# uzh-rpg/dagr

Measured on NVIDIA H100. Metric: Mevents/sec, higher is better.
Workload: dtype f32

## Files before the change

### dagr_b200/csrc/graph.cu

```cuda
#include "common.cuh"

#define SCAN_THREADS 256
#define SCAN_ITEMS 8
#define SCAN_TILE (SCAN_THREADS * SCAN_ITEMS)

extern "C" int64_t dagr_scan_blocks(int64_t n) { return (n + SCAN_TILE - 1) / SCAN_TILE; }

__global__ void __launch_bounds__(SCAN_THREADS) k_scan_reduce(const int *__restrict__ in, int64_t n, int *__restrict__ blocksums)
{
    __shared__ int sm[32];
    __shared__ int tot;
    int64_t base = (int64_t)blockIdx.x * SCAN_TILE + (int64_t)threadIdx.x * SCAN_ITEMS;
    int s = 0;
#pragma unroll
    for (int k = 0; k < SCAN_ITEMS; k++) { int64_t i = base + k; if (i < n) s += in[i]; }
    block_exclusive_scan(s, &tot, sm);
    if (threadIdx.x == 0) blocksums[blockIdx.x] = tot;
}

__global__ void __launch_bounds__(SCAN_THREADS) k_scan_blocksums(int *__restrict__ blocksums, int64_t nb)
{
    __shared__ int sm[32];
    __shared__ int tot;
    int carry = 0;
    for (int64_t c = 0; c < nb; c += SCAN_THREADS) {
        int64_t i = c + threadIdx.x;
        int v = (i < nb) ? blocksums[i] : 0;
        int ex = block_exclusive_scan(v, &tot, sm);
        if (i < nb) blocksums[i] = ex + carry;
        carry += tot;
        __syncthreads();
    }
    if (threadIdx.x == 0) blocksums[nb] = carry;
}

__global__ void __launch_bounds__(SCAN_THREADS) k_scan_apply(const int *__restrict__ in, int *__restrict__ out, int64_t n,
                                                             const int *__restrict__ blocksums, int64_t nb)
{
    __shared__ int sm[32];
    __shared__ int tot;
    int64_t base = (int64_t)blockIdx.x * SCAN_TILE + (int64_t)threadIdx.x * SCAN_ITEMS;
    int v[SCAN_ITEMS];
    int s = 0;
#pragma unroll
    for (int k = 0; k < SCAN_ITEMS; k++) { int64_t i = base + k; v[k] = (i < n) ? in[i] : 0; s += v[k]; }
    int ex = block_exclusive_scan(s, &tot, sm) + blocksums[blockIdx.x];
#pragma unroll
    for (int k = 0; k < SCAN_ITEMS; k++) { int64_t i = base + k; if (i < n) out[i] = ex; ex += v[k]; }
    if (blockIdx.x == 0 && threadIdx.x == 0) out[n] = blocksums[nb];
}

int scan_exclusive(const int *in, int *out, int64_t n, int *blocksums, cudaStream_t st)
{
    int64_t nb = dagr_scan_blocks(n);
    if (nb == 0) nb = 1;
    k_scan_reduce<<<(unsigned)nb, SCAN_THREADS, 0, st>>>(in, n, blocksums);
    k_scan_blocksums<<<1, SCAN_THREADS, 0, st>>>(blocksums, nb);
    k_scan_apply<<<(unsigned)nb, SCAN_THREADS, 0, st>>>(in, out, n, blocksums, nb);
    return 0;
}

__global__ void k_denorm(const float *__restrict__ pos, int64_t n3, float W, float H, float T, int32_t *__restrict__ out)
{
    int64_t i = (int64_t)blockIdx.x * blockDim.x + threadIdx.x;
    if (i >= n3) return;
    int d = (int)(i % 3);
    float s = d == 0 ? W : (d == 1 ? H : T);
    out[i] = (int)__fadd_rn(__fmul_rn(s, pos[i]), 1e-3f);
}

extern "C" int dagr_denormalize_pos(const float *pos, int64_t N, int W, int H, int T, int32_t *pos_i32, void *stream)
{
    if (N <= 0) return DAGR_OK;
    int64_t n3 = 3 * N;
    k_denorm<<<dagr_div_up(n3, 256), 256, 0, (cudaStream_t)stream>>>(pos, n3, (float)W, (float)H, (float)T, pos_i32);
    DAGR_CHECK_LAUNCH();
    return DAGR_OK;
}

__global__ void k_prepare_events(const float *__restrict__ pos, const int64_t *__restrict__ batch64, const float *__restrict__ x, int ldx,
                                 int64_t N, float W, float H, float T, int32_t *__restrict__ pos_i, int32_t *__restrict__ batch_i,
                                 float *__restrict__ feat)
{
    const int64_t i = (int64_t)blockIdx.x * blockDim.x + threadIdx.x;
    if (i >= N) return;
    pos_i[3 * i + 0] = (int)__fadd_rn(__fmul_rn(W, pos[3 * i + 0]), 1e-3f);
    pos_i[3 * i + 1] = (int)__fadd_rn(__fmul_rn(H, pos[3 * i + 1]), 1e-3f);
    pos_i[3 * i + 2] = (int)__fadd_rn(__fmul_rn(T, pos[3 * i + 2]), 1e-3f);
    batch_i[i] = (int32_t)batch64[i];
    feat[i] = x[i * ldx];
}

extern "C" int dagr_prepare_events(const float *pos, const int64_t *batch, const float *x, int ldx, int64_t N, int W, int H, int T,
                                   int32_t *pos_i32, int32_t *batch_i32, float *feat, void *stream)
{
    if (N <= 0) return DAGR_OK;
    DAGR_CHECK_ARG(pos && batch && x && pos_i32 && batch_i32 && feat && ldx >= 1, "bad argument");
    k_prepare_events<<<dagr_div_up(N, 256), 256, 0, (cudaStream_t)stream>>>(pos, batch, x, ldx, N, (float)W, (float)H, (float)T, pos_i32,
                                                                          batch_i32, feat);
    DAGR_CHECK_LAUNCH();
    return DAGR_OK;
}

struct RingAt {
    int64_t slot;
    int i;
};

__device__ __forceinline__ int64_t ring_total(const int32_t *ctl, int S, int64_t N)
{
    if (ctl == nullptr) return N;
    return S == 1 ? (int64_t)ctl[1] : (int64_t)ctl[DAGR_RING_CTL * S];
}

__device__ __forceinline__ RingAt ring_at(const int32_t *ctl, int S, int mask, int c)
{
    if (ctl == nullptr) return RingAt{(int64_t)c, c};
    int s = 0;
    if (S > 1) {
        int lo = 0, hi = S - 1;
        while (lo < hi) {
            const int mid = (lo + hi + 1) >> 1;
            if (__ldg(ctl + DAGR_RING_CTL * mid + 6) <= c) lo = mid; else hi = mid - 1;
        }
        s = lo;
    }
    const int32_t *cs = ctl + DAGR_RING_CTL * s;
    const int i = S > 1 ? c - __ldg(cs + 6) : c;
    return RingAt{(int64_t)s * (mask + 1) + ((__ldg(cs) + i) & mask), i};
}

__global__ void k_keys_hist(dagr_geom_t g, const int32_t *__restrict__ batch, const int32_t *__restrict__ pos, int64_t N,
                            int32_t *__restrict__ key, int32_t *__restrict__ count, int32_t *__restrict__ flags,
                            const int32_t *__restrict__ ctl, int mask, int S)
{
    int64_t i = (int64_t)blockIdx.x * blockDim.x + threadIdx.x;
    if (i >= ring_total(ctl, S, N)) return;
    const RingAt at = ring_at(ctl, S, mask, (int)i);
    const int64_t si = at.slot;
    int x = pos[3 * si], y = pos[3 * si + 1], b = batch[si];
    if (flags != nullptr && at.i > 0) {
        const int64_t sp = ctl != nullptr ? (si & ~(int64_t)mask) | ((si - 1) & mask) : si - 1;
        if (batch[sp] == b && pos[3 * sp + 2] > pos[3 * si + 2]) flags[0] = 1;
    }
    x = min(max(x, 0), g.W - 1); y = min(max(y, 0), g.H - 1); b = min(max(b, 0), g.B - 1);
    int k = b * (g.ny1 * g.nx1 * g.CP) + __ldg(g.ykey + y) + __ldg(g.xkey + x);
    key[i] = k;
    atomicAdd(count + k, 1);
}

__global__ void k_scatter(const int32_t *__restrict__ key, int64_t N, const int32_t *__restrict__ start,
                          int32_t *__restrict__ count, int32_t *__restrict__ tmp, const int32_t *__restrict__ ctl, int S)
{
    int64_t i = (int64_t)blockIdx.x * blockDim.x + threadIdx.x;
    if (i >= ring_total(ctl, S, N)) return;
    int k = key[i];
    int slot = atomicSub(count + k, 1) - 1;
    tmp[start[k] + slot] = (int)i;
}

__global__ void k_rank_emit(dagr_geom_t g, const int32_t *__restrict__ key, const int32_t *__restrict__ tmp, int64_t N,
                            const int32_t *__restrict__ start, const int32_t *__restrict__ batch,
                            const int32_t *__restrict__ pos, const float *__restrict__ feat,
                            int32_t *__restrict__ perm, int2 *__restrict__ ti, uint32_t *__restrict__ xyb,
                            float *__restrict__ feat_s, const int32_t *__restrict__ ctl, int mask, int S)
{
    int64_t j = (int64_t)blockIdx.x * blockDim.x + threadIdx.x;
    if (j >= ring_total(ctl, S, N)) return;
    int i = tmp[j];
    int k = key[i];
    int s = start[k], e = start[k + 1];
    int rank = 0;
    for (int q = s; q < e; q++) rank += (tmp[q] < i);
    int p = s + rank;
    const int64_t si = ring_at(ctl, S, mask, i).slot;
    int x = pos[3 * si], y = pos[3 * si + 1], t = pos[3 * si + 2], b = batch[si];
    x = min(max(x, 0), g.W - 1); y = min(max(y, 0), g.H - 1); b = min(max(b, 0), g.B - 1);
    perm[p] = i;
    ti[p] = make_int2(t, i);
    xyb[p] = (uint32_t)x | ((uint32_t)y << 12) | ((uint32_t)b << 24);
    feat_s[p] = feat[si];
}

static int graph_sort_impl(const dagr_geom_t *g, const int32_t *batch, const int32_t *pos, const float *feat,
                           int64_t N, const int32_t *ctl, int mask, int S, int32_t *key, int32_t *tmp, int32_t *count,
                           int32_t *blocksums, int32_t *start, int32_t *perm, int32_t *ti, uint32_t *xyb, float *feat_s,
                           int32_t *flags, void *stream)
{
    DAGR_CHECK_ARG(g && g->W <= 4096 && g->H <= 4096 && g->B <= 256, "geometry out of range (W,H<=4096, B<=256)");
    DAGR_CHECK_ARG(N >= 0 && N < (1ll << 31), "N out of range");
    cudaStream_t st = (cudaStream_t)stream;
    if (N > 0) {
        k_keys_hist<<<dagr_div_up(N, 256), 256, 0, st>>>(*g, batch, pos, N, key, count, flags, ctl, mask, S);
        DAGR_CHECK_LAUNCH();
    }
    scan_exclusive(count, start, g->NK, blocksums, st);
    DAGR_CHECK_LAUNCH();
    if (N > 0) {
        k_scatter<<<dagr_div_up(N, 256), 256, 0, st>>>(key, N, start, count, tmp, ctl, S);
        k_rank_emit<<<dagr_div_up(N, 256), 256, 0, st>>>(*g, key, tmp, N, start, batch, pos, feat, perm,
                                                         (int2 *)ti, xyb, feat_s, ctl, mask, S);
        DAGR_CHECK_LAUNCH();
    }
    return DAGR_OK;
}

extern "C" int dagr_graph_sort(const dagr_geom_t *g, const int32_t *batch, const int32_t *pos, const float *feat,
                               int64_t N, int32_t *key, int32_t *tmp, int32_t *count, int32_t *blocksums,
                               int32_t *start, int32_t *perm, int32_t *ti, uint32_t *xyb, float *feat_s,
                               int32_t *flags, void *stream)
{
    return graph_sort_impl(g, batch, pos, feat, N, nullptr, 0, 1, key, tmp, count, blocksums, start, perm, ti, xyb, feat_s, flags,
                           stream);
}

#define RING_MAX_STREAMS 128
static int check_rings(const char *who, int64_t capacity, int streams, int max_chunk)
{
    const char *msg = nullptr;
    if (streams < 1 || streams >= RING_MAX_STREAMS) msg = "streams must be in [1, 127]";
    else if (capacity <= 0 || (capacity & (capacity - 1)) != 0) msg = "ring capacity must be a power of two";
    else if ((int64_t)streams * capacity >= (1ll << 24)) msg = "streams * capacity must be < 2^24 (sorted positions are packed in 24 bits)";
    else if (max_chunk <= 0 || max_chunk > capacity) msg = "max_chunk must be in [1, capacity]";
    if (msg == nullptr) return DAGR_OK;
    dagr_set_error("%s: %s", who, msg);
    return DAGR_E_ARG;
}

extern "C" int dagr_graph_sort_ring(const dagr_geom_t *g, const int32_t *batch, const int32_t *pos, const float *feat,
                                    int64_t capacity, const int32_t *ctl, int32_t *key, int32_t *tmp, int32_t *count,
                                    int32_t *blocksums, int32_t *start, int32_t *perm, int32_t *ti, uint32_t *xyb, float *feat_s,
                                    int32_t *flags, void *stream)
{
    DAGR_CHECK_ARG(ctl != nullptr && capacity > 0 && (capacity & (capacity - 1)) == 0, "ring capacity must be a power of two");
    return graph_sort_impl(g, batch, pos, feat, capacity, ctl, (int)(capacity - 1), 1, key, tmp, count, blocksums, start, perm, ti,
                           xyb, feat_s, flags, stream);
}

extern "C" int dagr_graph_sort_rings(const dagr_geom_t *g, const int32_t *batch, const int32_t *pos, const float *feat,
                                     int64_t capacity, int streams, const int32_t *ctl, int32_t *key, int32_t *tmp, int32_t *count,
                                     int32_t *blocksums, int32_t *start, int32_t *perm, int32_t *ti, uint32_t *xyb, float *feat_s,
                                     int32_t *flags, void *stream)
{
    DAGR_CHECK_ARG(g && batch && pos && feat && ctl && key && tmp && count && blocksums && start && perm && ti && xyb && feat_s,
                   "null argument");
    const int rc = check_rings(__func__, capacity, streams, 1);
    if (rc != DAGR_OK) return rc;
    DAGR_CHECK_ARG(streams == g->B, "streams must equal the geometry's batch size B (stream s is sample s)");
    return graph_sort_impl(g, batch, pos, feat, (int64_t)streams * capacity, ctl, (int)(capacity - 1), streams, key, tmp, count,
                           blocksums, start, perm, ti, xyb, feat_s, flags, stream);
}

__global__ void __launch_bounds__(RING_MAX_STREAMS) k_stream_advance(int32_t *__restrict__ ctl, const int32_t *__restrict__ stage,
// ... 196 lines not shown
```

### dagr_b200/csrc/conv_l1.cu

```cuda
#include <string.h>
#include "common.cuh"

#define L1_THREADS 128

struct L1Smem {
    float *tab;
    float *posx;
    float *posy;
    short *sp;
};

__device__ __forceinline__ L1Smem l1_smem_init(const dagr_geom_t &g, const float *__restrict__ tab, unsigned char *raw)
{
    L1Smem s;
    s.tab = (float *)raw;
    s.posx = s.tab + g.ncell * DAGR_TABW;
    s.posy = s.posx + g.W;
    s.sp = (short *)(s.posy + g.H);
    for (int i = threadIdx.x; i < g.ncell * DAGR_TABW; i += blockDim.x) s.tab[i] = tab[i];
    for (int i = threadIdx.x; i < g.W; i += blockDim.x) s.posx[i] = g.posx0[i];
    for (int i = threadIdx.x; i < g.H; i += blockDim.x) s.posy[i] = g.posy0[i];
    for (int i = threadIdx.x; i < g.ncell; i += blockDim.x)
        s.sp[i] = (short)(((int)g.spiral[2 * i] & 0xff) | ((int)g.spiral[2 * i + 1] << 8));
    __syncthreads();
// ... 379 lines not shown
            const float4 wya = *reinterpret_cast<const float4 *>(wyb + yo);
            const float wy4 = *reinterpret_cast<const float *>(wy4b + (yo >> 2));
            CB2_EDGE_FMA();
        }
    } else {
#pragma unroll 1
        for (int q = -1; q < n; q++) {
            int row, dxi, dyi;
            if (q < 0) { row = p; dxi = r; dyi = r; }
            else {
                row = nbr[(int64_t)q * N + p];
                const uint32_t d = s_sp[off[(int64_t)q * N + p]];
                dxi = (int)(d & 31u); dyi = (int)(d >> 5);
            }
            const int sw = XA_SWZ(row);
            const float4 *src = reinterpret_cast<const float4 *>(xa + ((int64_t)half * N + row) * 8);
            const float4 t0 = src[sw], t1 = src[sw ^ 1];
            const float wx = s_wx[grp * 32 + dxi];
            const float4 wya = s_wy[dyi];
            const float wy4 = s_wy4[dyi];
            CB2_EDGE_FMA();
        }
    }
#undef CB2_EDGE_FMA
    if constexpr (TC) {
        const float4 *wf = wfrag + ((size_t)half * CB2_TC_KSTEPS * 32 + (threadIdx.x & 31)) * 2;
        float2 c2[8];
#pragma unroll
        for (int i = 0; i < 8; i++) c2[i] = make_float2(0.f, 0.f);
#pragma unroll
        for (int j = 0; j < CB2_G; j++) {
            const float a[8] = {A[j][0].x, A[j][0].y, A[j][1].x, A[j][1].y, A[j][2].x, A[j][2].y, A[j][3].x, A[j][3].y};
            cb2_tc_kstep(xt, a, wf + (grp + 3 * j) * 64, c2);
        }
#pragma unroll
        for (int i = 0; i < 8; i++) o2[i] = make_float2(__fadd_rn(o2[i].x, c2[i].x), __fadd_rn(o2[i].y, c2[i].y));
        return;
    }
#pragma unroll
    for (int j = 0; j < CB2_G; j++)
#pragma unroll
        for (int k = 0; k < 4; k++)
#pragma unroll
            for (int c4 = 0; c4 < 4; c4++) {
                const float4 wa = *reinterpret_cast<const float4 *>(&P.w[grp + 3 * j][8 * half + 2 * k][4 * c4]);
                const float4 wb = *reinterpret_cast<const float4 *>(&P.w[grp + 3 * j][8 * half + 2 * k + 1][4 * c4]);
                o2[2 * c4] = ffma2(make_float2(A[j][k].x, A[j][k].x), make_float2(wa.x, wa.y), o2[2 * c4]);
                o2[2 * c4 + 1] = ffma2(make_float2(A[j][k].x, A[j][k].x), make_float2(wa.z, wa.w), o2[2 * c4 + 1]);
                o2[2 * c4] = ffma2(make_float2(A[j][k].y, A[j][k].y), make_float2(wb.x, wb.y), o2[2 * c4]);
                o2[2 * c4 + 1] = ffma2(make_float2(A[j][k].y, A[j][k].y), make_float2(wb.z, wb.w), o2[2 * c4 + 1]);
            }
}

__device__ __forceinline__ float cb2_div_floor(float a, float b)
{
    const float mod = fmodf(a, b);
    float div = __fdiv_rn(__fsub_rn(a, mod), b);
    if ((mod != 0.f) && ((b < 0.f) != (mod < 0.f))) div -= 1.f;
    float fl;
    if (div != 0.f) { fl = floorf(div); if (div - fl > 0.5f) fl += 1.f; }
    else fl = copysignf(0.f, __fdiv_rn(a, b));
    return fl;
}
__device__ __forceinline__ int cb2_round_to_pixel(float mean, int size)
{
    const float inv = __frcp_rn((float)size);
    const int k = (int)cb2_div_floor(__fadd_rn(mean, 1e-5f), inv);
    return min(max(k, 0), size - 1);
}

template <int THREADS>
struct CB2Shared {
    CB2Tile T;
    uint64_t bar;
    float red[THREADS / 32][16];
    long long sum[THREADS / 32][3];
    int tm[THREADS / 32];
    __align__(16) float xt[THREADS / 32][64];
};

template <class PT, int NCH, bool MODE_A, int CAP, int THREADS, bool POOL_MEAN, bool PLAIN, bool TC>
__device__ __forceinline__ void cb2_voxel(const dagr_geom_t &g, int64_t N, const int32_t *__restrict__ start, const uint32_t *__restrict__ xyb,
             const int2 *__restrict__ ti, const float *__restrict__ feat_s, const float *__restrict__ xa,
             const int32_t *__restrict__ nbr, const uint16_t *__restrict__ off,
             const PT &P, const float4 *__restrict__ wfrag, const float *__restrict__ skip_pre_in, const int min_idx_in,
             float *__restrict__ persist_in, float *__restrict__ x1_in, int32_t *__restrict__ cnt, int32_t *__restrict__ pxy,
             float *__restrict__ tmean, float *__restrict__ tmax, float *__restrict__ xg, int ldx,
             float *__restrict__ xa_out, float *__restrict__ skip_out,
             const int cell, unsigned char *smem_raw, CB2Shared<THREADS> &S, uint32_t &parity,
             int32_t *__restrict__ wl_hdr, int32_t *__restrict__ wl_ids, const int defer)
{
    const int min_idx = PLAIN ? 0 : min_idx_in;
    float *const persist = PLAIN ? nullptr : persist_in;
    float *const x1 = PLAIN ? nullptr : x1_in;
    const float *const skip_pre = PLAIN ? nullptr : skip_pre_in;
    const bool relu = PLAIN ? true : (P.relu != 0);
    CB2Tile &T = S.T;
    uint64_t &s_bar = S.bar;
    auto &s_red = S.red;
    auto &s_sum = S.sum;
    auto &s_tm = S.tm;
    float *const xt = S.xt[threadIdx.x >> 5];
    float *s_rows = (float *)smem_raw;
    float *s_wx = s_rows + (size_t)CAP * 8;
    float4 *s_wy = (float4 *)(s_wx + 128);
    float *s_wy4 = (float *)(s_wy + 32);
    uint32_t *s_ell = (uint32_t *)(s_wy + 64);
    uint16_t *s_sp = (uint16_t *)(s_ell + DAGR_ELL * THREADS);
    const int per = g.ny1 * g.nx1;
    const int b = cell / per, rem = cell % per, cy = rem / g.nx1, cx = rem % g.nx1;
    const int p0 = start[(int64_t)cell * g.CP], p1 = start[(int64_t)(cell + 1) * g.CP];
    const int nown = p1 - p0;
    if (nown == 0) {
        if (MODE_A) return;
        if (threadIdx.x == 0) { cnt[cell] = 0; pxy[2 * cell] = 0; pxy[2 * cell + 1] = 0; tmean[cell] = 0.f; tmax[cell] = 0.f; }
        if (threadIdx.x < 16) xg[(int64_t)cell * ldx + threadIdx.x] = 0.f;
        return;
    }
    if (threadIdx.x < 32) {
        const int clo = max(cx - 1, 0), chi = min(cx + 1, g.nx1 - 1);
        const int lane = threadIdx.x, rr = lane >> 1, ry = cy - 1 + rr;
        int v = 0;
        if (lane < 6 && ry >= 0 && ry < g.ny1)
            v = start[((int64_t)b * per + ry * g.nx1 + ((lane & 1) ? chi + 1 : clo)) * g.CP];
        int o = 0;
#pragma unroll
        for (int k = 0; k < 3; k++) {
            const int s0 = __shfl_sync(0xffffffffu, v, 2 * k), e0 = __shfl_sync(0xffffffffu, v, 2 * k + 1);
            const bool ok = (cy - 1 + k >= 0) && (cy - 1 + k < g.ny1);
            if (lane == 0) { T.run_start[k] = ok ? s0 : 0; T.run_len[k] = ok ? e0 - s0 : 0; T.run_off[k] = o; }
            o += ok ? e0 - s0 : 0;
        }
    }
    for (int i = threadIdx.x; i < 2 * g.r + 1; i += blockDim.x) {
        const float4 tx = __ldg(reinterpret_cast<const float4 *>(g.tabx) + i);
        s_wx[i] = tx.x; s_wx[32 + i] = tx.y; s_wx[64 + i] = tx.z;
        s_wy[i] = __ldg(reinterpret_cast<const float4 *>(g.taby) + 2 * i);
        s_wy4[i] = __ldg(g.taby + 8 * i + 4);
    }
    for (int i = threadIdx.x; i < g.ncell; i += blockDim.x)
        s_sp[i] = (uint16_t)(((int)g.spiral[2 * i] + g.r) | (((int)g.spiral[2 * i + 1] + g.r) << 5));
    __syncthreads();
    const int total = T.run_off[2] + T.run_len[2];
    const bool staged = total <= CAP;
    if (!staged && wl_hdr != nullptr) {
        int slot = 0;
        if (threadIdx.x == 0) slot = atomicAdd(&wl_hdr[0], 1);
        if (defer) { if (threadIdx.x == 0) wl_ids[slot] = cell; return; }
    }
    const int s1 = T.run_start[1];
    const int s2 = T.run_len[2] > 0 ? T.run_start[2] : 0x7fffffff;
    const int d0 = T.run_off[0] - T.run_start[0], d1 = T.run_off[1] - T.run_start[1], d2 = T.run_off[2] - T.run_start[2];

    constexpr bool pool_mean = POOL_MEAN && !MODE_A;
    float m[16];
#pragma unroll
    for (int c = 0; c < 16; c++) m[c] = pool_mean ? 0.f : -INFINITY;
    long long sx = 0, sy = 0, st = 0;
    int tm = -2147483647;
    const bool sparse = MODE_A && staged && nown <= 32;
    const int lane_ = threadIdx.x & 31, wid_ = threadIdx.x >> 5;
    for (int pb0 = p0; pb0 < p1; pb0 += blockDim.x) {
        const int p = sparse ? p0 + lane_ : pb0 + threadIdx.x;
        const bool inrange = sparse ? (p < p1 && wid_ < 3) : (p < p1);
        const int tix = sparse ? lane_ : (int)threadIdx.x;
        const bool active = inrange && (min_idx <= 0 || ti[p].y >= min_idx);
        if (min_idx > 0 && !__syncthreads_or(active)) {
            if (inrange) { const uint32_t w0 = xyb[p]; const int t0 = ti[p].x; sx += w0 & 0xfff; sy += (w0 >> 12) & 0xfff; st += t0; tm = max(tm, t0); }
            continue;
        }
        const int n = active ? nbr[(int64_t)(DAGR_ELL - 1) * N + p] : 0;
        if (staged && active && (!sparse || wid_ == 0)) {
            int jj[DAGR_ELL - 1]; int cc[DAGR_ELL - 1];
#pragma unroll
            for (int q = 0; q < DAGR_ELL - 1; q++) {
                jj[q] = (q < n) ? nbr[(int64_t)q * N + p] : 0;
                cc[q] = (q < n) ? (int)off[(int64_t)q * N + p] : 0;
            }
#pragma unroll
            for (int q = 0; q < DAGR_ELL - 1; q++) {
                const int j = jj[q];
                const int row = j + (j >= s2 ? d2 : (j >= s1 ? d1 : d0));
                s_ell[(q + 1) * THREADS + tix] = ((uint32_t)(2 * row + XA_SWZ(j)) << 4) | ((uint32_t)s_sp[cc[q]] << 18);
            }
            s_ell[tix] = ((uint32_t)(2 * (p + d1) + XA_SWZ(p)) << 4) | ((uint32_t)(g.r | (g.r << 5)) << 18);
        }
        float2 o2[8], sk2[MODE_A ? 8 : 1];
#pragma unroll
        for (int k = 0; k < 8; k++) o2[k] = make_float2(0.f, 0.f);
#pragma unroll
        for (int k = 0; k < (MODE_A ? 8 : 1); k++) sk2[k] = make_float2(0.f, 0.f);
#pragma unroll 1
        for (int half = 0; half < NCH; half++) {
            if (staged) {
                __syncthreads();
                if (threadIdx.x == 0) {
                    mbar_expect_tx(&s_bar, (uint32_t)total * 32u);
                    for (int rr = 0; rr < 3; rr++)
                        if (T.run_len[rr] > 0)
                            tma_bulk_g2s(s_rows + (size_t)T.run_off[rr] * 8, xa + ((size_t)half * N + T.run_start[rr]) * 8,
                                         (uint32_t)T.run_len[rr] * 32u, &s_bar);
                }
                mbar_wait(&s_bar, parity);
                parity ^= 1;
            }
            if (TC ? __any_sync(0xffffffffu, active) : active) {
                const int nn = active ? n : -1;
#define CB2_ROOT(H)                                                                                                  \
    do {                                                                                                            \
        const float4 *src = staged ? reinterpret_cast<const float4 *>(s_rows + (int64_t)(p + d1) * 8)               \
                                   : reinterpret_cast<const float4 *>(xa + ((int64_t)(H) * N + p) * 8);             \
        const float4 z4 = make_float4(0.f, 0.f, 0.f, 0.f);                                                         \
        const float4 t0 = active ? src[XA_SWZ(p)] : z4, t1 = active ? src[XA_SWZ(p) ^ 1] : z4;                      \
        const float v[8] = {t0.x, t0.y, t0.z, t0.w, t1.x, t1.y, t1.z, t1.w};                                        \
        if constexpr (TC) {                                                                                         \
            float2 c2[8];                                                                                           \
            _Pragma("unroll") for (int i = 0; i < 8; i++) c2[i] = make_float2(0.f, 0.f);                            \
            cb2_tc_kstep(xt, v, wfrag + (((H) * CB2_TC_KSTEPS + 15) * 32 + lane_) * 2, c2);                         \
            _Pragma("unroll") for (int i = 0; i < 8; i++)                                                           \
                o2[i] = make_float2(__fadd_rn(o2[i].x, c2[i].x), __fadd_rn(o2[i].y, c2[i].y));                      \
        }                                                                                                           \
        _Pragma("unroll") for (int k = 0; k < 8; k++)                                                               \
            _Pragma("unroll") for (int c4 = 0; c4 < 4; c4++) {                                                      \
                if constexpr (!TC) {                                                                                \
                    const float4 w4 = *reinterpret_cast<const float4 *>(&P.root[8 * (H) + k][4 * c4]);              \
                    o2[2 * c4] = ffma2(make_float2(v[k], v[k]), make_float2(w4.x, w4.y), o2[2 * c4]);               \
                    o2[2 * c4 + 1] = ffma2(make_float2(v[k], v[k]), make_float2(w4.z, w4.w), o2[2 * c4 + 1]);       \
                }                                                                                                   \
                if constexpr (MODE_A) {                     \
                    const float4 k4 = *reinterpret_cast<const float4 *>(&P.skip[8 * (H) + k][4 * c4]);              \
                    sk2[2 * c4] = ffma2(make_float2(v[k], v[k]), make_float2(k4.x, k4.y), sk2[2 * c4]);             \
                    sk2[2 * c4 + 1] = ffma2(make_float2(v[k], v[k]), make_float2(k4.z, k4.w), sk2[2 * c4 + 1]);     \
                }                                                                                                   \
            }                                                                                                       \
    } while (0)
                if (!sparse || wid_ == 0) {
                    if (half == 0)      CB2_ROOT(0);
                    else if (half == 1) CB2_ROOT(1);
                    else if constexpr (NCH > 2) CB2_ROOT(2);
                }
#undef CB2_ROOT
#define CB2_PASS(H, G)                                                                                               \
    do {                                                                                                            \
        if (staged) cb2_pass<true, H, G, THREADS, TC>(N, p, nn, xa, s_rows, s_wx, s_wy, s_wy4, s_ell, s_sp, nbr, off, P, wfrag, xt, p + d1, g.r, tix, o2); \
        else        cb2_pass<false, H, G, THREADS, TC>(N, p, nn, xa, s_rows, s_wx, s_wy, s_wy4, s_ell, s_sp, nbr, off, P, wfrag, xt, 0, g.r, tix, o2);     \
    } while (0)
#define CB2_HALF(H)                                                                                                  \
    do {                                                                                                            \
        if (!sparse) { CB2_PASS(H, 0); CB2_PASS(H, 1); CB2_PASS(H, 2); }                                            \
        else if (wid_ == 0) CB2_PASS(H, 0);                                                                         \
        else if (wid_ == 1) CB2_PASS(H, 1);                                                                         \
        else CB2_PASS(H, 2);                                                                                        \
    } while (0)
                if (half == 0)      CB2_HALF(0);
                else if (half == 1) CB2_HALF(1);
                else if constexpr (NCH > 2) CB2_HALF(2);
#undef CB2_HALF
#undef CB2_PASS
            }
        }
        if constexpr (TC) {
            if (__any_sync(0xffffffffu, active)) cb2_tc_unfrag(xt, o2);
        }
        if (sparse) {
            __syncthreads();
            float *s_part = s_rows;
            if (active && wid_ >= 1) {
                float4 *dst = reinterpret_cast<float4 *>(s_part + ((size_t)(wid_ - 1) * 32 + lane_) * 16);
                dst[0] = make_float4(o2[0].x, o2[0].y, o2[1].x, o2[1].y);
                dst[1] = make_float4(o2[2].x, o2[2].y, o2[3].x, o2[3].y);
                dst[2] = make_float4(o2[4].x, o2[4].y, o2[5].x, o2[5].y);
                dst[3] = make_float4(o2[6].x, o2[6].y, o2[7].x, o2[7].y);
            }
            __syncthreads();
            if (active && wid_ == 0) {
#pragma unroll
                for (int w2 = 0; w2 < 2; w2++) {
                    const float4 *src = reinterpret_cast<const float4 *>(s_part + ((size_t)w2 * 32 + lane_) * 16);
#pragma unroll
                    for (int k = 0; k < 4; k++) {
                        const float4 v = src[k];
                        o2[2 * k].x += v.x; o2[2 * k].y += v.y; o2[2 * k + 1].x += v.z; o2[2 * k + 1].y += v.w;
                    }
                }
            }
        }
        const bool owner = !sparse || wid_ == 0;
        if (!MODE_A && inrange && owner) { const uint32_t w0 = xyb[p]; const int t0 = ti[p].x; sx += w0 & 0xfff; sy += (w0 >> 12) & 0xfff; st += t0; tm = max(tm, t0); }
        if (!active || !owner) continue;
        float o[16];
#pragma unroll
        for (int c = 0; c < 8; c++) { o[2 * c] = o2[c].x; o[2 * c + 1] = o2[c].y; }
        if constexpr (MODE_A) {
            float sk[16];
#pragma unroll
            for (int c = 0; c < 8; c++) { sk[2 * c] = sk2[c].x; sk[2 * c + 1] = sk2[c].y; }
            const int sw = XA_SWZ(p);
            {
                const float4 *pp = reinterpret_cast<const float4 *>(xa_out + (int64_t)p * 8);
                const float4 a0 = pp[sw], a1 = pp[sw ^ 1];
                pp = reinterpret_cast<const float4 *>(xa_out + (N + (int64_t)p) * 8);
                const float4 a2 = pp[sw], a3 = pp[sw ^ 1];
// ... 57 lines not shown
            float4 *dst = reinterpret_cast<float4 *>(x1 + (int64_t)p * 16);
            dst[0] = make_float4(o[0], o[1], o[2], o[3]);
            dst[1] = make_float4(o[4], o[5], o[6], o[7]);
            dst[2] = make_float4(o[8], o[9], o[10], o[11]);
            dst[3] = make_float4(o[12], o[13], o[14], o[15]);
        }
    }
    if (MODE_A) return;
    const int lane = threadIdx.x & 31, wid = threadIdx.x >> 5;
#pragma unroll
    for (int d = 16; d > 0; d >>= 1) {
#pragma unroll
        for (int c = 0; c < 16; c++) {
            const float o2 = __shfl_xor_sync(0xffffffffu, m[c], d);
            m[c] = pool_mean ? m[c] + o2 : fmaxf(m[c], o2);
        }
        sx += __shfl_xor_sync(0xffffffffu, sx, d);
        sy += __shfl_xor_sync(0xffffffffu, sy, d);
        st += __shfl_xor_sync(0xffffffffu, st, d);
        tm = max(tm, __shfl_xor_sync(0xffffffffu, tm, d));
    }
    if (lane == 0) {
#pragma unroll
        for (int c = 0; c < 16; c++) s_red[wid][c] = m[c];
        s_sum[wid][0] = sx; s_sum[wid][1] = sy; s_sum[wid][2] = st; s_tm[wid] = tm;
    }
    __syncthreads();
    const int nw = blockDim.x >> 5;
    if (threadIdx.x < 16) {
        float v = s_red[0][threadIdx.x];
        for (int w2 = 1; w2 < nw; w2++) v = pool_mean ? v + s_red[w2][threadIdx.x] : fmaxf(v, s_red[w2][threadIdx.x]);
        if (pool_mean) v = __fdiv_rn(v, (float)nown);
        if (persist != nullptr) {
            if (min_idx > 0) v = fmaxf(v, persist[(int64_t)cell * 16 + threadIdx.x]);
            persist[(int64_t)cell * 16 + threadIdx.x] = v;
        }
        xg[(int64_t)cell * ldx + threadIdx.x] = v;
    }
    if (threadIdx.x == 32) {
        long long ax = 0, ay = 0, at = 0; int tmx = -2147483647;
        for (int w2 = 0; w2 < nw; w2++) { ax += s_sum[w2][0]; ay += s_sum[w2][1]; at += s_sum[w2][2]; tmx = max(tmx, s_tm[w2]); }
        const float mx = (float)((double)ax / ((double)nown * (double)g.W));
        const float my = (float)((double)ay / ((double)nown * (double)g.H));
        cnt[cell] = nown;
        pxy[2 * cell] = cb2_round_to_pixel(mx, g.W);
        pxy[2 * cell + 1] = cb2_round_to_pixel(my, g.H);
        tmean[cell] = (float)((double)at / ((double)nown * (double)g.T));
        tmax[cell] = __fdiv_rn((float)tmx, (float)g.T);
    }
}


template <class PT, int NCH, bool MODE_A, bool POOL_MEAN, bool PLAIN, bool TC>
__global__ void __launch_bounds__(CB2_THREADS, MODE_A ? 3 : 4)
k_l1_conv_b2(const dagr_geom_t g, int64_t N, const int32_t *__restrict__ start, const uint32_t *__restrict__ xyb,
             const int2 *__restrict__ ti, const float *__restrict__ feat_s, const float *__restrict__ xa,
             const int32_t *__restrict__ nbr, const uint16_t *__restrict__ off,
             const __grid_constant__ PT P, const float4 *__restrict__ wfrag, const float *__restrict__ skip_pre, const int min_idx,
             float *__restrict__ persist, float *__restrict__ x1, int32_t *__restrict__ cnt, int32_t *__restrict__ pxy,
             float *__restrict__ tmean, float *__restrict__ tmax, float *__restrict__ xg, int ldx,
             float *__restrict__ xa_out, float *__restrict__ skip_out, int32_t *__restrict__ wl_hdr, int32_t *__restrict__ wl_ids,
             const int defer)
{
    extern __shared__ __align__(128) unsigned char smem_raw[];
    __shared__ __align__(16) CB2Shared<CB2_THREADS> S;
    if (threadIdx.x == 0) mbar_init(&S.bar, 1);
    uint32_t parity = 0;
    cb2_voxel<PT, NCH, MODE_A, CB2_CAP, CB2_THREADS, POOL_MEAN, PLAIN, TC>(g, N, start, xyb, ti, feat_s, xa, nbr, off, P, wfrag, skip_pre, min_idx,
                                                      persist, x1, cnt, pxy, tmean, tmax, xg, ldx, xa_out, skip_out, (int)blockIdx.x,
                                                      smem_raw, S, parity, wl_hdr, wl_ids, defer);
}

template <class PT, int NCH, bool MODE_A, bool POOL_MEAN, bool PLAIN, bool TC>
__global__ void __launch_bounds__(CB2_THREADS_BIG, 1)
k_l1_conv_b2_dense(const dagr_geom_t g, int64_t N, const int32_t *__restrict__ start, const uint32_t *__restrict__ xyb,
                   const int2 *__restrict__ ti, const float *__restrict__ feat_s, const float *__restrict__ xa,
                   const int32_t *__restrict__ nbr, const uint16_t *__restrict__ off,
                   const __grid_constant__ PT P, const float4 *__restrict__ wfrag, const float *__restrict__ skip_pre, const int min_idx,
                   float *__restrict__ persist, float *__restrict__ x1, int32_t *__restrict__ cnt, int32_t *__restrict__ pxy,
                   float *__restrict__ tmean, float *__restrict__ tmax, float *__restrict__ xg, int ldx,
                   float *__restrict__ xa_out, float *__restrict__ skip_out, int32_t *__restrict__ wl_hdr, const int32_t *__restrict__ wl_ids)
{
    extern __shared__ __align__(128) unsigned char smem_raw[];
    __shared__ __align__(16) CB2Shared<CB2_THREADS_BIG> S;
    __shared__ int s_next;
    if (threadIdx.x == 0) mbar_init(&S.bar, 1);
    uint32_t parity = 0;
    const int count = wl_hdr[0];
    for (;;) {
        __syncthreads();
        if (threadIdx.x == 0) s_next = atomicAdd(&wl_hdr[1], 1);
        __syncthreads();
        const int i = s_next;
        if (i >= count) break;
        cb2_voxel<PT, NCH, MODE_A, CB2_CAP_BIG, CB2_THREADS_BIG, POOL_MEAN, PLAIN, TC>(g, N, start, xyb, ti, feat_s, xa, nbr, off, P, wfrag, skip_pre,
                                                                  min_idx, persist, x1, cnt, pxy, tmean, tmax, xg, ldx, xa_out, skip_out,
                                                                  wl_ids[i], smem_raw, S, parity, nullptr, nullptr, 0);
    }
}

static size_t cb2_smem_bytes(const dagr_geom_t *g, int cap, int threads)
{
    return (size_t)cap * 32 + 96 * 16 + (size_t)DAGR_ELL * threads * 4 + (size_t)g->ncell * 2 + 32;
}

template <class PT, int NCH, bool MODE_A, bool TC, bool POOL_MEAN = false, bool PLAIN = false>
static int cb2_launch(const dagr_geom_t *g, int64_t N, const int32_t *start, const uint32_t *xyb, const int2 *ti, const float *feat_s,
// ... 164 lines not shown
```

Before: 576.2.

## Vectorize scan I/O and fold bucket cursors into scan output

Scan kernels now load and store each thread's eight items as two int4 accesses when aligned and in bounds. The scan apply step also writes per-bucket end cursors back into the count array, so scatter needs one atomicSub and no lookup of start. The rank/emit kernel resets count to zero per bucket, which may let later calls skip a separate memset, and derives the batch index from the key instead of reading it. The cost is more coupling between kernels: count now carries state from one stage to the next, and in-place aliasing drops the __restrict__ qualifiers.

```diff
diff --git a/dagr_b200/csrc/graph.cu b/dagr_b200/csrc/graph.cu
--- a/dagr_b200/csrc/graph.cu
+++ b/dagr_b200/csrc/graph.cu
@@ -6,14 +6,44 @@
 
 extern "C" int64_t dagr_scan_blocks(int64_t n) { return (n + SCAN_TILE - 1) / SCAN_TILE; }
 
-__global__ void __launch_bounds__(SCAN_THREADS) k_scan_reduce(const int *__restrict__ in, int64_t n, int *__restrict__ blocksums)
+static_assert(SCAN_ITEMS == 8, "a thread's items are two int4");
+
+__device__ __forceinline__ bool scan_vec(const void *p, int64_t base, int64_t n)
+{
+    return base + SCAN_ITEMS <= n && ((uintptr_t)p & 15) == 0;
+}
+__device__ __forceinline__ void scan_load(const int *p, int64_t base, int64_t n, int v[SCAN_ITEMS])
+{
+    if (scan_vec(p, base, n)) {
+        const int4 a = *reinterpret_cast<const int4 *>(p + base), b = *reinterpret_cast<const int4 *>(p + base + 4);
+        v[0] = a.x; v[1] = a.y; v[2] = a.z; v[3] = a.w; v[4] = b.x; v[5] = b.y; v[6] = b.z; v[7] = b.w;
+    } else {
+#pragma unroll
+        for (int k = 0; k < SCAN_ITEMS; k++) v[k] = base + k < n ? p[base + k] : 0;
+    }
+}
+__device__ __forceinline__ void scan_store(int *p, int64_t base, int64_t n, const int v[SCAN_ITEMS])
+{
+    if (scan_vec(p, base, n)) {
+        *reinterpret_cast<int4 *>(p + base) = make_int4(v[0], v[1], v[2], v[3]);
+        *reinterpret_cast<int4 *>(p + base + 4) = make_int4(v[4], v[5], v[6], v[7]);
+    } else {
+#pragma unroll
+        for (int k = 0; k < SCAN_ITEMS; k++)
+            if (base + k < n) p[base + k] = v[k];
+    }
+}
+
+__global__ void __launch_bounds__(SCAN_THREADS) k_scan_reduce(const int *in, int64_t n, int *__restrict__ blocksums)
 {
     __shared__ int sm[32];
     __shared__ int tot;
     int64_t base = (int64_t)blockIdx.x * SCAN_TILE + (int64_t)threadIdx.x * SCAN_ITEMS;
+    int v[SCAN_ITEMS];
+    scan_load(in, base, n, v);
     int s = 0;
 #pragma unroll
-    for (int k = 0; k < SCAN_ITEMS; k++) { int64_t i = base + k; if (i < n) s += in[i]; }
+    for (int k = 0; k < SCAN_ITEMS; k++) s += v[k];
     block_exclusive_scan(s, &tot, sm);
     if (threadIdx.x == 0) blocksums[blockIdx.x] = tot;
 }
@@ -34,29 +64,41 @@
     if (threadIdx.x == 0) blocksums[nb] = carry;
 }
 
-__global__ void __launch_bounds__(SCAN_THREADS) k_scan_apply(const int *__restrict__ in, int *__restrict__ out, int64_t n,
-                                                             const int *__restrict__ blocksums, int64_t nb)
+__global__ void __launch_bounds__(SCAN_THREADS) k_scan_apply(const int *in, int *out, int64_t n, const int *__restrict__ blocksums,
+                                                             int64_t nb, int *cursor)
 {
     __shared__ int sm[32];
     __shared__ int tot;
     int64_t base = (int64_t)blockIdx.x * SCAN_TILE + (int64_t)threadIdx.x * SCAN_ITEMS;
-    int v[SCAN_ITEMS];
+    int v[SCAN_ITEMS], o[SCAN_ITEMS];
+    scan_load(in, base, n, v);
     int s = 0;
 #pragma unroll
-    for (int k = 0; k < SCAN_ITEMS; k++) { int64_t i = base + k; v[k] = (i < n) ? in[i] : 0; s += v[k]; }
+    for (int k = 0; k < SCAN_ITEMS; k++) s += v[k];
     int ex = block_exclusive_scan(s, &tot, sm) + blocksums[blockIdx.x];
 #pragma unroll
-    for (int k = 0; k < SCAN_ITEMS; k++) { int64_t i = base + k; if (i < n) out[i] = ex; ex += v[k]; }
+    for (int k = 0; k < SCAN_ITEMS; k++) { o[k] = ex; ex += v[k]; }
+    scan_store(out, base, n, o);
+    if (cursor != nullptr) {
+#pragma unroll
+        for (int k = 0; k < SCAN_ITEMS; k++) o[k] = v[k] > 0 ? o[k] + v[k] : 0;
+        scan_store(cursor, base, n, o);
+    }
     if (blockIdx.x == 0 && threadIdx.x == 0) out[n] = blocksums[nb];
 }
 
-int scan_exclusive(const int *in, int *out, int64_t n, int *blocksums, cudaStream_t st)
+static void scan_launch(const int *in, int *out, int64_t n, int *blocksums, int *cursor, cudaStream_t st)
 {
     int64_t nb = dagr_scan_blocks(n);
     if (nb == 0) nb = 1;
     k_scan_reduce<<<(unsigned)nb, SCAN_THREADS, 0, st>>>(in, n, blocksums);
     k_scan_blocksums<<<1, SCAN_THREADS, 0, st>>>(blocksums, nb);
-    k_scan_apply<<<(unsigned)nb, SCAN_THREADS, 0, st>>>(in, out, n, blocksums, nb);
+    k_scan_apply<<<(unsigned)nb, SCAN_THREADS, 0, st>>>(in, out, n, blocksums, nb, cursor);
+}
+
+int scan_exclusive(const int *in, int *out, int64_t n, int *blocksums, cudaStream_t st)
+{
+    scan_launch(in, out, n, blocksums, nullptr, st);
     return 0;
 }
 
@@ -149,18 +191,16 @@
     atomicAdd(count + k, 1);
 }
 
-__global__ void k_scatter(const int32_t *__restrict__ key, int64_t N, const int32_t *__restrict__ start,
-                          int32_t *__restrict__ count, int32_t *__restrict__ tmp, const int32_t *__restrict__ ctl, int S)
+__global__ void k_scatter(const int32_t *__restrict__ key, int64_t N, int32_t *__restrict__ count, int32_t *__restrict__ tmp,
+                          const int32_t *__restrict__ ctl, int S)
 {
     int64_t i = (int64_t)blockIdx.x * blockDim.x + threadIdx.x;
     if (i >= ring_total(ctl, S, N)) return;
-    int k = key[i];
-    int slot = atomicSub(count + k, 1) - 1;
-    tmp[start[k] + slot] = (int)i;
+    tmp[atomicSub(count + key[i], 1) - 1] = (int)i;
 }
 
 __global__ void k_rank_emit(dagr_geom_t g, const int32_t *__restrict__ key, const int32_t *__restrict__ tmp, int64_t N,
-                            const int32_t *__restrict__ start, const int32_t *__restrict__ batch,
+                            const int32_t *__restrict__ start, int32_t *__restrict__ count,
                             const int32_t *__restrict__ pos, const float *__restrict__ feat,
                             int32_t *__restrict__ perm, int2 *__restrict__ ti, uint32_t *__restrict__ xyb,
                             float *__restrict__ feat_s, const int32_t *__restrict__ ctl, int mask, int S)
@@ -173,9 +213,11 @@
     int rank = 0;
     for (int q = s; q < e; q++) rank += (tmp[q] < i);
     int p = s + rank;
+    if (rank == 0) count[k] = 0;
     const int64_t si = ring_at(ctl, S, mask, i).slot;
-    int x = pos[3 * si], y = pos[3 * si + 1], t = pos[3 * si + 2], b = batch[si];
-    x = min(max(x, 0), g.W - 1); y = min(max(y, 0), g.H - 1); b = min(max(b, 0), g.B - 1);
+    int x = pos[3 * si], y = pos[3 * si + 1], t = pos[3 * si + 2];
+    const int b = k / (g.ny1 * g.nx1 * g.CP);
+    x = min(max(x, 0), g.W - 1); y = min(max(y, 0), g.H - 1);
     perm[p] = i;
     ti[p] = make_int2(t, i);
     xyb[p] = (uint32_t)x | ((uint32_t)y << 12) | ((uint32_t)b << 24);
@@ -194,11 +236,11 @@
         k_keys_hist<<<dagr_div_up(N, 256), 256, 0, st>>>(*g, batch, pos, N, key, count, flags, ctl, mask, S);
         DAGR_CHECK_LAUNCH();
     }
-    scan_exclusive(count, start, g->NK, blocksums, st);
+    scan_launch(count, start, g->NK, blocksums, count, st);
     DAGR_CHECK_LAUNCH();
     if (N > 0) {
-        k_scatter<<<dagr_div_up(N, 256), 256, 0, st>>>(key, N, start, count, tmp, ctl, S);
-        k_rank_emit<<<dagr_div_up(N, 256), 256, 0, st>>>(*g, key, tmp, N, start, batch, pos, feat, perm,
+        k_scatter<<<dagr_div_up(N, 256), 256, 0, st>>>(key, N, count, tmp, ctl, S);
+        k_rank_emit<<<dagr_div_up(N, 256), 256, 0, st>>>(*g, key, tmp, N, start, count, pos, feat, perm,
                                                          (int2 *)ti, xyb, feat_s, ctl, mask, S);
         DAGR_CHECK_LAUNCH();
     }
```

Result: faster. 584.1, median of 6 (+1.4%).

## Split each event's neighbor gather across lane pairs for the tensor-core L1 conv path

Applied to the files above, without the earlier changes.

Adds a paired-lane path for the staged, tensor-core, non-mode-A case. Each event's gathered neighbor rows are split across two lanes that each handle half of the channels. The path runs two 16-row m-tiles per warp, staging accumulators through a larger swizzled per-warp shared buffer and loading them with ldmatrix x4 before the 3xTF32 MMAs. It also lowers the minimum CTAs per SM in launch bounds from 4 to 3 so the larger register and shared-memory footprint fits. The aim is better lane utilisation and fewer shared-memory transposes, at the cost of lower occupancy and more per-lane loop iterations.

```diff
diff --git a/dagr_b200/csrc/conv_l1.cu b/dagr_b200/csrc/conv_l1.cu
--- a/dagr_b200/csrc/conv_l1.cu
+++ b/dagr_b200/csrc/conv_l1.cu
@@ -455,6 +455,120 @@
             }
 }
 
+#ifndef CB2_LANES
+#define CB2_LANES 2
+#endif
+#ifndef CB2_MIN_CTAS
+#define CB2_MIN_CTAS 3
+#endif
+#ifndef CB2_XT_FLOATS
+#define CB2_XT_FLOATS (CB2_MIN_CTAS >= 4 ? 64 : 128)
+#endif
+template <int half, int THREADS>
+__device__ __forceinline__ void cb2_pair_mtile(int n, int col, const float *s_rows, const float4 *s_wx4, const float4 *s_wy,
+                                               const float *s_wy4, const uint32_t *s_ell, const float4 *__restrict__ wfrag, float *xt,
+                                               float2 c[4])
+{
+    const int lane = threadIdx.x & 31, h = lane & 1;
+    float4 A[DAGR_KU];
+#pragma unroll
+    for (int u = 0; u < DAGR_KU; u++) A[u] = make_float4(0.f, 0.f, 0.f, 0.f);
+    const char *rb = reinterpret_cast<const char *>(s_rows), *wxb = reinterpret_cast<const char *>(s_wx4);
+    const char *wyb = reinterpret_cast<const char *>(s_wy), *wy4b = reinterpret_cast<const char *>(s_wy4);
+    const uint32_t hx = 16u * (uint32_t)h;
+#pragma unroll 1
+    for (int q = 0; q <= n; q++) {
+        const uint32_t ell = s_ell[q * THREADS + col];
+        const uint32_t ro = (ell & 0x3fff0u) ^ hx, xo = (ell >> 14) & 0x1f0u, yo = (ell >> 19) & 0x1f0u;
+        const float4 e = *reinterpret_cast<const float4 *>(rb + ro);
+        const float4 wx4 = *reinterpret_cast<const float4 *>(wxb + xo);
+        const float4 wya = *reinterpret_cast<const float4 *>(wyb + yo);
+        const float wy4 = *reinterpret_cast<const float *>(wy4b + (yo >> 2));
+        const float wx[3] = {wx4.x, wx4.y, wx4.z};
+        const float wy[CB2_G] = {wya.x, wya.y, wya.z, wya.w, wy4};
+#pragma unroll
+        for (int k = 0; k < 3; k++)
+#pragma unroll
+            for (int j = 0; j < CB2_G; j++) {
+                const float w = __fmul_rn(wy[j], wx[k]);
+                float4 &a = A[k + 3 * j];
+                a.x = fmaf(w, e.x, a.x); a.y = fmaf(w, e.y, a.y); a.z = fmaf(w, e.z, a.z); a.w = fmaf(w, e.w, a.w);
+            }
+    }
+    const float4 *wf = wfrag + ((size_t)half * CB2_TC_KSTEPS * 32 + lane) * 2;
+#if CB2_XT_FLOATS >= 128
+    const int i_ = lane >> 1, mrow = 8 * ((lane >> 3) & 1) + (lane & 7), mch = lane >> 4;
+    float *row = xt + 8 * i_ + 4 * (h ^ ((i_ >> 2) & 1));
+    const uint32_t ra = smem_u32(xt + 8 * mrow + 4 * (mch ^ ((mrow >> 2) & 1)));
+#else
+    float *row = xt + 4 * (lane >> 1);
+    const uint32_t ra = smem_u32(xt + 4 * (lane & 15));
+#endif
+#pragma unroll
+    for (int grp = 0; grp < 3; grp++) {
+        float2 c2[4];
+#pragma unroll
+        for (int i = 0; i < 4; i++) c2[i] = make_float2(0.f, 0.f);
+#pragma unroll
+        for (int j = 0; j < CB2_G; j++) {
+            const int u = grp + 3 * j;
+            const float4 w0 = __ldg(wf + u * 64), w1 = __ldg(wf + u * 64 + 1);
+            const uint32_t bh[2][2] = {{__float_as_uint(w0.x), __float_as_uint(w0.y)}, {__float_as_uint(w1.x), __float_as_uint(w1.y)}};
+            const uint32_t bl[2][2] = {{__float_as_uint(w0.z), __float_as_uint(w0.w)}, {__float_as_uint(w1.z), __float_as_uint(w1.w)}};
+            uint32_t ah[4], al[4];
+#if CB2_XT_FLOATS >= 128
+            __syncwarp();
+            *reinterpret_cast<float4 *>(row) = A[u];
+            __syncwarp();
+            ldsm_x4(ra, ah);
+#pragma unroll
+            for (int i = 0; i < 4; i++) tf32_split(ah[i], ah[i], al[i]);
+#else
+#pragma unroll
+            for (int hh = 0; hh < 2; hh++) {
+                __syncwarp();
+                if (h == hh) *reinterpret_cast<float4 *>(row) = A[u];
+                __syncwarp();
+                uint32_t r0, r1;
+                ldsm_x2(ra, r0, r1);
+                tf32_split(r0, ah[2 * hh], al[2 * hh]);
+                tf32_split(r1, ah[2 * hh + 1], al[2 * hh + 1]);
+            }
+#endif
+#pragma unroll
+            for (int nt = 0; nt < 2; nt++) {
+                mma_tf32(c2[2 * nt], c2[2 * nt + 1], al, bh[nt][0], bh[nt][1]);
+                mma_tf32(c2[2 * nt], c2[2 * nt + 1], ah, bl[nt][0], bl[nt][1]);
+                mma_tf32(c2[2 * nt], c2[2 * nt + 1], ah, bh[nt][0], bh[nt][1]);
+            }
+        }
+#pragma unroll
+        for (int i = 0; i < 4; i++) c[i] = make_float2(__fadd_rn(c[i].x, c2[i].x), __fadd_rn(c[i].y, c2[i].y));
+    }
+}
+
+template <int half, int THREADS>
+__device__ __forceinline__ void cb2_pair_half(int nn, const float *s_rows, const float4 *s_wx4, const float4 *s_wy, const float *s_wy4,
+                                              const uint32_t *s_ell, const float4 *__restrict__ wfrag, float *xt, float2 o2[8])
+{
+    const int lane = threadIdx.x & 31;
+#pragma unroll 1
+    for (int mt = 0; mt < 2; mt++) {
+        const int src = 16 * mt + (lane >> 1);
+        const int n = __shfl_sync(0xffffffffu, nn, src);
+        if (!__any_sync(0xffffffffu, n >= 0)) continue;
+        float2 c[4];
+#pragma unroll
+        for (int i = 0; i < 4; i++) c[i] = mt ? o2[4 + i] : o2[i];
+        cb2_pair_mtile<half, THREADS>(n, (int)(threadIdx.x & ~31u) + src, s_rows, s_wx4, s_wy, s_wy4, s_ell, wfrag, xt, c);
+#pragma unroll
+        for (int i = 0; i < 4; i++) {
+            if (mt) o2[4 + i] = c[i];
+            else o2[i] = c[i];
+        }
+    }
+}
+
 __device__ __forceinline__ float cb2_div_floor(float a, float b)
 {
     const float mod = fmodf(a, b);
@@ -479,7 +593,7 @@
     float red[THREADS / 32][16];
     long long sum[THREADS / 32][3];
     int tm[THREADS / 32];
-    __align__(16) float xt[THREADS / 32][64];
+    __align__(16) float xt[THREADS / 32][CB2_XT_FLOATS];
 };
 
 template <class PT, int NCH, bool MODE_A, int CAP, int THREADS, bool POOL_MEAN, bool PLAIN, bool TC>
@@ -505,9 +619,10 @@
     auto &s_tm = S.tm;
     float *const xt = S.xt[threadIdx.x >> 5];
     float *s_rows = (float *)smem_raw;
-    float *s_wx = s_rows + (size_t)CAP * 8;
-    float4 *s_wy = (float4 *)(s_wx + 128);
+    float4 *s_wx4 = (float4 *)(s_rows + (size_t)CAP * 8);
+    float4 *s_wy = s_wx4 + 32;
     float *s_wy4 = (float *)(s_wy + 32);
+    float *s_wx = s_wy4 + 32;
     uint32_t *s_ell = (uint32_t *)(s_wy + 64);
     uint16_t *s_sp = (uint16_t *)(s_ell + DAGR_ELL * THREADS);
     const int per = g.ny1 * g.nx1;
@@ -538,6 +653,7 @@
     for (int i = threadIdx.x; i < 2 * g.r + 1; i += blockDim.x) {
         const float4 tx = __ldg(reinterpret_cast<const float4 *>(g.tabx) + i);
         s_wx[i] = tx.x; s_wx[32 + i] = tx.y; s_wx[64 + i] = tx.z;
+        s_wx4[i] = make_float4(tx.x, tx.y, tx.z, 0.f);
         s_wy[i] = __ldg(reinterpret_cast<const float4 *>(g.taby) + 2 * i);
         s_wy4[i] = __ldg(g.taby + 8 * i + 4);
     }
@@ -562,6 +678,7 @@
     long long sx = 0, sy = 0, st = 0;
     int tm = -2147483647;
     const bool sparse = MODE_A && staged && nown <= 32;
+    constexpr bool kPair = CB2_LANES == 2 && TC && !MODE_A;
     const int lane_ = threadIdx.x & 31, wid_ = threadIdx.x >> 5;
     for (int pb0 = p0; pb0 < p1; pb0 += blockDim.x) {
         const int p = sparse ? p0 + lane_ : pb0 + threadIdx.x;
@@ -650,7 +767,8 @@
     } while (0)
 #define CB2_HALF(H)                                                                                                  \
     do {                                                                                                            \
-        if (!sparse) { CB2_PASS(H, 0); CB2_PASS(H, 1); CB2_PASS(H, 2); }                                            \
+        if (kPair && staged) cb2_pair_half<H, THREADS>(nn, s_rows, s_wx4, s_wy, s_wy4, s_ell, wfrag, xt, o2);      \
+        else if (!sparse) { CB2_PASS(H, 0); CB2_PASS(H, 1); CB2_PASS(H, 2); }                                       \
         else if (wid_ == 0) CB2_PASS(H, 0);                                                                         \
         else if (wid_ == 1) CB2_PASS(H, 1);                                                                         \
         else CB2_PASS(H, 2);                                                                                        \
@@ -814,7 +932,7 @@
 
 
 template <class PT, int NCH, bool MODE_A, bool POOL_MEAN, bool PLAIN, bool TC>
-__global__ void __launch_bounds__(CB2_THREADS, MODE_A ? 3 : 4)
+__global__ void __launch_bounds__(CB2_THREADS, MODE_A ? 3 : CB2_MIN_CTAS)
 k_l1_conv_b2(const dagr_geom_t g, int64_t N, const int32_t *__restrict__ start, const uint32_t *__restrict__ xyb,
              const int2 *__restrict__ ti, const float *__restrict__ feat_s, const float *__restrict__ xa,
              const int32_t *__restrict__ nbr, const uint16_t *__restrict__ off,
```

After: 577.2 before, 594.5 after (median of 6 runs). 3.0% higher.

## Fuse scan apply with count reset and simplify scatter via cursor counters

Applied to the files above, without the earlier changes.

Replaces the generic exclusive scan with a sort-specific apply kernel. It writes start offsets with vectorized int4 stores and turns the count array into per-bucket cursors. Scatter then needs only one atomicAdd and one tmp write, without reading start. The rank/emit kernel recomputes the key from pos instead of reading key[], and resets count to zero for the next call, so a separate memset is no longer needed. The catch is that correctness now depends on count being zeroed by rank 0 of each bucket, with extra ykey/xkey lookups.

```diff
diff --git a/dagr_b200/csrc/graph.cu b/dagr_b200/csrc/graph.cu
--- a/dagr_b200/csrc/graph.cu
+++ b/dagr_b200/csrc/graph.cu
@@ -149,18 +149,50 @@
     atomicAdd(count + k, 1);
 }
 
-__global__ void k_scatter(const int32_t *__restrict__ key, int64_t N, const int32_t *__restrict__ start,
-                          int32_t *__restrict__ count, int32_t *__restrict__ tmp, const int32_t *__restrict__ ctl, int S)
+__global__ void __launch_bounds__(SCAN_THREADS) k_sort_scan_apply(int32_t *__restrict__ count, int32_t *__restrict__ start, int64_t n,
+                                                                  const int32_t *__restrict__ blocksums, int64_t nb)
+{
+    __shared__ int sm[32];
+    __shared__ int tot;
+    const int64_t base = (int64_t)blockIdx.x * SCAN_TILE + (int64_t)threadIdx.x * SCAN_ITEMS;
+    const bool vec = ((reinterpret_cast<uintptr_t>(count) | reinterpret_cast<uintptr_t>(start)) & 15) == 0 && base + SCAN_ITEMS <= n;
+    int v[SCAN_ITEMS];
+    if (vec) {
+        const int4 a = reinterpret_cast<const int4 *>(count + base)[0], b = reinterpret_cast<const int4 *>(count + base)[1];
+        v[0] = a.x; v[1] = a.y; v[2] = a.z; v[3] = a.w; v[4] = b.x; v[5] = b.y; v[6] = b.z; v[7] = b.w;
+    } else {
+#pragma unroll
+        for (int k = 0; k < SCAN_ITEMS; k++) v[k] = base + k < n ? count[base + k] : 0;
+    }
+    int s = 0;
+#pragma unroll
+    for (int k = 0; k < SCAN_ITEMS; k++) s += v[k];
+    int ex = block_exclusive_scan(s, &tot, sm) + blocksums[blockIdx.x];
+    int o[SCAN_ITEMS];
+#pragma unroll
+    for (int k = 0; k < SCAN_ITEMS; k++) { o[k] = ex; ex += v[k]; }
+    if (vec) {
+        reinterpret_cast<int4 *>(start + base)[0] = make_int4(o[0], o[1], o[2], o[3]);
+        reinterpret_cast<int4 *>(start + base)[1] = make_int4(o[4], o[5], o[6], o[7]);
+    } else {
+#pragma unroll
+        for (int k = 0; k < SCAN_ITEMS; k++) if (base + k < n) start[base + k] = o[k];
+    }
+#pragma unroll
+    for (int k = 0; k < SCAN_ITEMS; k++) if (v[k] != 0) count[base + k] = o[k];
+    if (blockIdx.x == 0 && threadIdx.x == 0) start[n] = blocksums[nb];
+}
+
+__global__ void k_scatter(const int32_t *__restrict__ key, int64_t N, int32_t *__restrict__ count, int32_t *__restrict__ tmp,
+                          const int32_t *__restrict__ ctl, int S)
 {
     int64_t i = (int64_t)blockIdx.x * blockDim.x + threadIdx.x;
     if (i >= ring_total(ctl, S, N)) return;
-    int k = key[i];
-    int slot = atomicSub(count + k, 1) - 1;
-    tmp[start[k] + slot] = (int)i;
-}
-
-__global__ void k_rank_emit(dagr_geom_t g, const int32_t *__restrict__ key, const int32_t *__restrict__ tmp, int64_t N,
-                            const int32_t *__restrict__ start, const int32_t *__restrict__ batch,
+    tmp[atomicAdd(count + key[i], 1)] = (int)i;
+}
+
+__global__ void k_rank_emit(dagr_geom_t g, const int32_t *__restrict__ tmp, int64_t N,
+                            const int32_t *__restrict__ start, int32_t *__restrict__ count, const int32_t *__restrict__ batch,
                             const int32_t *__restrict__ pos, const float *__restrict__ feat,
                             int32_t *__restrict__ perm, int2 *__restrict__ ti, uint32_t *__restrict__ xyb,
                             float *__restrict__ feat_s, const int32_t *__restrict__ ctl, int mask, int S)
@@ -168,14 +200,15 @@
     int64_t j = (int64_t)blockIdx.x * blockDim.x + threadIdx.x;
     if (j >= ring_total(ctl, S, N)) return;
     int i = tmp[j];
-    int k = key[i];
+    const int64_t si = ring_at(ctl, S, mask, i).slot;
+    int x = pos[3 * si], y = pos[3 * si + 1], t = pos[3 * si + 2], b = batch[si];
+    x = min(max(x, 0), g.W - 1); y = min(max(y, 0), g.H - 1); b = min(max(b, 0), g.B - 1);
+    const int k = b * (g.ny1 * g.nx1 * g.CP) + __ldg(g.ykey + y) + __ldg(g.xkey + x);
     int s = start[k], e = start[k + 1];
     int rank = 0;
     for (int q = s; q < e; q++) rank += (tmp[q] < i);
+    if (rank == 0) count[k] = 0;
     int p = s + rank;
-    const int64_t si = ring_at(ctl, S, mask, i).slot;
-    int x = pos[3 * si], y = pos[3 * si + 1], t = pos[3 * si + 2], b = batch[si];
-    x = min(max(x, 0), g.W - 1); y = min(max(y, 0), g.H - 1); b = min(max(b, 0), g.B - 1);
     perm[p] = i;
     ti[p] = make_int2(t, i);
     xyb[p] = (uint32_t)x | ((uint32_t)y << 12) | ((uint32_t)b << 24);
@@ -194,11 +227,14 @@
         k_keys_hist<<<dagr_div_up(N, 256), 256, 0, st>>>(*g, batch, pos, N, key, count, flags, ctl, mask, S);
         DAGR_CHECK_LAUNCH();
     }
-    scan_exclusive(count, start, g->NK, blocksums, st);
+    const int64_t nb = dagr_scan_blocks(g->NK) > 0 ? dagr_scan_blocks(g->NK) : 1;
+    k_scan_reduce<<<(unsigned)nb, SCAN_THREADS, 0, st>>>(count, g->NK, blocksums);
+    k_scan_blocksums<<<1, SCAN_THREADS, 0, st>>>(blocksums, nb);
+    k_sort_scan_apply<<<(unsigned)nb, SCAN_THREADS, 0, st>>>(count, start, g->NK, blocksums, nb);
     DAGR_CHECK_LAUNCH();
     if (N > 0) {
-        k_scatter<<<dagr_div_up(N, 256), 256, 0, st>>>(key, N, start, count, tmp, ctl, S);
-        k_rank_emit<<<dagr_div_up(N, 256), 256, 0, st>>>(*g, key, tmp, N, start, batch, pos, feat, perm,
+        k_scatter<<<dagr_div_up(N, 256), 256, 0, st>>>(key, N, count, tmp, ctl, S);
+        k_rank_emit<<<dagr_div_up(N, 256), 256, 0, st>>>(*g, tmp, N, start, count, batch, pos, feat, perm,
                                                          (int2 *)ti, xyb, feat_s, ctl, mask, S);
         DAGR_CHECK_LAUNCH();
     }
```

Result: no change. 579.2 before, 584.9 after (median of 6 runs) (+1.0%).
